# glmanhtu/vit-ed

Hardware: AMD Instinct MI355X
Metric: patch-pairs/sec fwd+bwd, div2k_erosion7_4bin_patch8_64 ViT-ED (higher is better)
Workload: dtype bf16

## Files before the change

### include/vited.h

```cpp
#ifndef VITED_H
#define VITED_H

#include <stdint.h>

#ifdef __cplusplus
extern "C" {
#endif

#define VITED_ABI_VERSION 1

#define VITED_OK 0
#define VITED_ERR_BAD_ARG 1
#define VITED_ERR_UNSUPPORTED 2
#define VITED_ERR_LAUNCH 3
#define VITED_ERR_WORKSPACE 4

#define VITED_F32 0
#define VITED_BF16 1
#define VITED_F16 2
#define VITED_I32 3
#define VITED_I64 4

#define VITED_EPI_STORE 0
#define VITED_EPI_GELU 1
// ... 112 lines not shown
int vited_qk_norm_fwd(const void* q, int64_t q_ld, int64_t q_rows, const void* k, int64_t k_ld, int64_t k_rows,
                      const float* gamma_q, const float* beta_q, const float* gamma_k, const float* beta_k, void* q_out,
                      int64_t q_out_ld, void* k_out, int64_t k_out_ld, float* q_mean, float* q_rstd, float* k_mean,
                      float* k_rstd, int dtype, int64_t heads, int64_t head_dim, float eps, void* stream);

int64_t vited_qk_norm_bwd_workspace_bytes(int64_t q_rows, int64_t k_rows, int64_t heads, int64_t head_dim);
int vited_qk_norm_bwd(void* dq, int64_t dq_ld, const void* q, int64_t q_ld, const float* q_mean, const float* q_rstd,
                      const float* gamma_q, float* dgamma_q, float* dbeta_q, int64_t q_rows, void* dk, int64_t dk_ld,
                      const void* k, int64_t k_ld, const float* k_mean, const float* k_rstd, const float* gamma_k,
                      float* dgamma_k, float* dbeta_k, int64_t k_rows, int dtype, int accumulate, int64_t heads,
                      int64_t head_dim, float* workspace, int64_t workspace_bytes, void* stream);


int64_t vited_token_pool_workspace_bytes(int64_t items, int64_t tokens, int64_t first, int64_t dim);
int vited_token_pool_fwd(const float* x, int64_t x_is, int64_t x_ts, const float* gamma, const float* beta, float eps,
                         float* pooled, int64_t pooled_ld, float* mean, float* rstd, int64_t items, int64_t tokens,
                         int64_t first, int64_t dim, float* workspace, int64_t workspace_bytes, void* stream);

int vited_token_pool_bwd(const float* g, int64_t g_ld, const float* x, int64_t x_is, int64_t x_ts, const float* gamma,
                         const float* mean, const float* rstd, float* dx, int64_t dx_is, int64_t dx_ts, void* dx_lp,
                         int dx_lp_dtype, int64_t dx_lp_is, int64_t dx_lp_ts, const float* lp_scale, float* dgamma,
                         float* dbeta, int accumulate, int64_t items, int64_t tokens, int64_t first, int64_t dim,
                         float* workspace, int64_t workspace_bytes, void* stream);


int vited_gemm(const void* A, int64_t lda, const void* B, int64_t ldb, int b_layout, int dtype, int64_t M,
               int64_t N, int64_t K, int epilogue, const float* bias, const void* aux,
               const float* residual, void* out, void* out2, int64_t ldo, int64_t rows_per_batch,
               int64_t out_rows_per_batch, int64_t row_offset, int residual_bcast, void* stream);

int vited_gemm_scaled(const void* A, int64_t lda, const void* B, int64_t ldb, int b_layout, int dtype, int64_t M, int64_t N,
                      int64_t K, const float* bias, const float* residual, const float* row_scale, float* out, int64_t ldo,
                      void* stream);

int64_t vited_linear_bwd_weight_workspace_bytes(int64_t M, int64_t N, int64_t K);
int vited_linear_bwd_weight(const void* dY, int64_t lddy, const void* X, int64_t ldx, int dtype, int64_t M,
                            int64_t N, int64_t K, float* dW, float* dbias, int accumulate, float* workspace,
                            int64_t workspace_bytes, void* stream);

int vited_linear_bwd_weight_batched_supported(int count, const int64_t* M, const int64_t* N, const int64_t* K, int dtype);
int64_t vited_linear_bwd_weight_batched_workspace_bytes(int count, const int64_t* M, const int64_t* N, const int64_t* K);
int vited_linear_bwd_weight_batched(int count, const void* const* dY, const int64_t* lddy, const void* const* X,
                                    const int64_t* ldx, const int64_t* M, const int64_t* N, const int64_t* K, float* const* dW,
                                    float* const* dbias, int dtype, int accumulate, float* workspace, int64_t workspace_bytes,
                                    void* stream);

int vited_linear_layernorm_supported(int64_t M, int64_t N, int64_t K);

int vited_linear_residual_layernorm_fwd(const void* a, int64_t lda, const void* w, int64_t ldw, const float* bias,
                                        const float* residual, int64_t ldr, float* y, int64_t ldy, const float* gamma,
                                        const float* beta, float eps, void* h, int64_t ldh, float* mean, float* rstd,
                                        int64_t M, int64_t N, int64_t K, void* stream);

int vited_linear_residual_layernorm_fwd_scaled(const void* a, int64_t lda, const void* w, int64_t ldw, const float* bias,
                                               const float* residual, int64_t ldr, const float* row_scale, float* y, int64_t ldy,
                                               const float* gamma, const float* beta, float eps, void* h, int64_t ldh, float* mean,
                                               float* rstd, int64_t M, int64_t N, int64_t K, void* stream);

int vited_linear_layernorm_bwd_segmented(const void* dy, int64_t lddy, int64_t seg_k, int64_t seg_stride, int64_t segments,
                                         const void* wt, int64_t ldwt, const float* x, int64_t ldx, const float* gamma,
                                         const float* mean, const float* rstd, const float* dx_in, int64_t dx_in_ld,
                                         float* dx_out, int64_t dx_out_ld, void* dx_lp, int64_t dx_lp_ld, float* dgamma,
                                         float* dbeta, int accumulate, int64_t M, int64_t N, float* workspace,
                                         int64_t workspace_bytes, void* stream);
int64_t vited_linear_layernorm_bwd_partial_rows(int64_t M);
int64_t vited_linear_layernorm_bwd_partial_rows_n(int64_t M, int64_t N);
// ... 202 lines not shown
```

### vit-ed_amd/csrc/gemm.hip

```cpp
#include <stdlib.h>
#include <string.h>

#include "gemm_kernels.h"

static thread_local int g_last_gemm_path = 0;
extern "C" int vited_last_gemm_path(void) { return g_last_gemm_path; }

static thread_local int g_last_fp32_gemm_kernel = 0;
static int g_fp32_gemm_select = 0;
extern "C" int vited_last_fp32_gemm_kernel(void) { return g_last_fp32_gemm_kernel; }
extern "C" int vited_fp32_gemm_select(int mode) {
    if (mode != 0 && mode != 1) return VITED_ERR_BAD_ARG;
    return __atomic_exchange_n(&g_fp32_gemm_select, mode, __ATOMIC_RELAXED);
}
extern "C" int vited_gemm_f32_mfma_supported(int64_t M, int64_t N, int64_t K, int b_layout, int epilogue) {
    if (M <= 0 || N <= 0 || K <= 0 || epilogue < VITED_EPI_STORE || epilogue > VITED_EPI_GELU_GRAD) return 0;
    return gemm_f32_mfma_supported(M, N, K, b_layout, epilogue) ? 1 : 0;
}
static inline bool fp32_gemm_on_matrix_cores(int64_t M, int64_t N, int64_t K, int b_layout, int epilogue) {
    return __atomic_load_n(&g_fp32_gemm_select, __ATOMIC_RELAXED) == 0 && gemm_f32_mfma_supported(M, N, K, b_layout, epilogue);
}

static int gemm_impl(const void* A, int64_t lda, const void* B, int64_t ldb, int b_layout, int dtype, int64_t M, int64_t N, int64_t K,
                     int epilogue, const float* bias, const void* aux, const float* residual, void* out, void* out2, int64_t ldo,
// ... 21 lines not shown
    ep.out2 = out2;
    ep.ldo = ldo;
    ep.rows_per_batch = epilogue == VITED_EPI_RESIDUAL ? rows_per_batch : 0;
    ep.out_rows_per_batch = out_rows_per_batch;
    ep.row_offset = row_offset;
    ep.residual_bcast = residual_bcast;
    hipStream_t s = (hipStream_t)stream;
    if (dtype == VITED_BF16 && b_layout == VITED_B_NK && gemm_nt_mfma_supported(A, lda, B, ldb, M, N, K, epilogue, ep)) {
        g_last_gemm_path = 2;
        return gemm_nt_mfma(A, lda, B, ldb, M, N, K, epilogue, ep, s);
    }
    g_last_gemm_path = 1;
    if (fp32_gemm_on_matrix_cores(M, N, K, b_layout, epilogue)) {
        g_last_fp32_gemm_kernel = 2;
        return gemm_f32_mfma(A, lda, B, ldb, b_layout, dtype, M, N, K, epilogue, ep, s);
    }
    g_last_fp32_gemm_kernel = 1;
    return gemm_portable(A, lda, B, ldb, b_layout, dtype, M, N, K, epilogue, ep, s);
}

extern "C" int vited_gemm(const void* A, int64_t lda, const void* B, int64_t ldb, int b_layout, int dtype, int64_t M,
                          int64_t N, int64_t K, int epilogue, const float* bias, const void* aux, const float* residual,
                          void* out, void* out2, int64_t ldo, int64_t rows_per_batch, int64_t out_rows_per_batch,
                          int64_t row_offset, int residual_bcast, void* stream) {
    return gemm_impl(A, lda, B, ldb, b_layout, dtype, M, N, K, epilogue, bias, aux, residual, out, out2, ldo, rows_per_batch,
                     out_rows_per_batch, row_offset, residual_bcast, nullptr, stream);
}

extern "C" int vited_gemm_scaled(const void* A, int64_t lda, const void* B, int64_t ldb, int b_layout, int dtype, int64_t M,
                                 int64_t N, int64_t K, const float* bias, const float* residual, const float* row_scale,
                                 float* out, int64_t ldo, void* stream) {
    return gemm_impl(A, lda, B, ldb, b_layout, dtype, M, N, K, VITED_EPI_RESIDUAL, bias, nullptr, residual, out, nullptr, ldo, 0, 0, 0, 0,
                     row_scale, stream);
}

static inline int64_t tn_portable_splits(int64_t M, int64_t N, int64_t K) {
    const int64_t tiles = ceil_div64(N, 64) * ceil_div64(K, 64);
    int64_t s = ceil_div64(1024, tiles);
    const int64_t max_s = ceil_div64(M, 256);
    if (s > max_s) s = max_s;
    if (s < 1) s = 1;
    const int64_t rps = ceil_div64(ceil_div64(M, s), 16) * 16;
    return ceil_div64(M, rps);
}

static inline int64_t max64(int64_t a, int64_t b) { return a > b ? a : b; }

extern "C" int64_t vited_linear_bwd_weight_workspace_bytes(int64_t M, int64_t N, int64_t K) {
    const int64_t s = max64(tn_portable_splits(M, N, K), gemm_tn_mfma_splits(M, N, K));
    return (s * N * K + s * N + N) * (int64_t)sizeof(float) + vited_sum_rows_workspace_bytes(M, N) + 256;
}

extern "C" int vited_linear_bwd_weight(const void* dY, int64_t lddy, const void* X, int64_t ldx, int dtype, int64_t M,
                                       int64_t N, int64_t K, float* dW, float* dbias, int accumulate, float* workspace,
                                       int64_t workspace_bytes, void* stream) {
    if (!dY || !X || !dW || M <= 0 || N <= 0 || K <= 0 || lddy < N || ldx < K) return VITED_ERR_BAD_ARG;
    if (dtype != VITED_F32 && dtype != VITED_BF16) return VITED_ERR_UNSUPPORTED;
    if (!workspace || workspace_bytes < vited_linear_bwd_weight_workspace_bytes(M, N, K)) return VITED_ERR_WORKSPACE;
    hipStream_t s = (hipStream_t)stream;
    const bool mfma = dtype == VITED_BF16 && gemm_tn_mfma_supported(dY, lddy, X, ldx, M, N, K);
    const int64_t splits = mfma ? gemm_tn_mfma_splits(M, N, K) : tn_portable_splits(M, N, K);
    const bool via_slabs = splits > 1 || accumulate;
    float* slab = via_slabs ? workspace : dW;
    float* bias_tmp = workspace + splits * N * K;
    int rc;
    if (mfma) {
// ... 74 lines not shown
```

### vit-ed_amd/csrc/gemm_kernels.h

```cpp
#pragma once
#include "gemm_epilogue.h"

int gemm_portable(const void* A, int64_t lda, const void* B, int64_t ldb, int b_layout, int dtype, int64_t M, int64_t N,
                  int64_t K, int epilogue, const EpiParams& ep, hipStream_t s);
int gemm_tn_portable(const void* dY, int64_t lddy, const void* X, int64_t ldx, int dtype, int64_t M, int64_t N, int64_t K,
                     int64_t splits, float* out, hipStream_t s);

bool gemm_f32_mfma_supported(int64_t M, int64_t N, int64_t K, int b_layout, int epilogue);
int gemm_f32_mfma(const void* A, int64_t lda, const void* B, int64_t ldb, int b_layout, int dtype, int64_t M, int64_t N,
                  int64_t K, int epilogue, const EpiParams& ep, hipStream_t s);
int gemm_tn_f32_mfma(const void* dY, int64_t lddy, const void* X, int64_t ldx, int dtype, int64_t M, int64_t N, int64_t K,
                     int64_t splits, float* out, hipStream_t s);

bool gemm_nt_mfma_supported(const void* A, int64_t lda, const void* B, int64_t ldb, int64_t M, int64_t N, int64_t K,
                            int epilogue, const EpiParams& ep);
int gemm_nt_mfma(const void* A, int64_t lda, const void* B, int64_t ldb, int64_t M, int64_t N, int64_t K, int epilogue,
                 const EpiParams& ep, hipStream_t s);
bool gemm_nt_areg_supported(int64_t ldw, int64_t M, int64_t N, int64_t K, int epilogue);
int gemm_nt_areg(const void* A, int64_t lda, const void* W, int64_t ldw, int64_t M, int64_t N, int epilogue, int waves,
                 const EpiParams& ep, hipStream_t s);
bool gemm_tn_mfma_supported(const void* dY, int64_t lddy, const void* X, int64_t ldx, int64_t M, int64_t N, int64_t K);
int64_t gemm_tn_mfma_splits(int64_t M, int64_t N, int64_t K);
int gemm_tn_mfma(const void* dY, int64_t lddy, const void* X, int64_t ldx, int64_t M, int64_t N, int64_t K, int64_t splits,
                 float* out, float* bias_out , hipStream_t s);

bool gemm_tn_batch_supported(int count, const int64_t* M, const int64_t* N, const int64_t* K);
void gemm_tn_batch_layout(int count, const int64_t* M, const int64_t* N, const int64_t* K, int64_t* splits, int64_t* slab_stride,
                          int64_t* bias_stride);
int gemm_tn_batch(int count, const void* const* dY, const int64_t* lddy, const void* const* X, const int64_t* ldx, const int64_t* M,
                  const int64_t* N, const int64_t* K, const int* has_bias, float* slabs, float* bias_slabs, hipStream_t s);
int sum_slabs_batch(int count, const float* slabs, int64_t slab_stride, const float* bias_slabs, int64_t bias_stride, int64_t splits,
                    const int64_t* widths, float* const* dW, const int64_t* nbias, float* const* dbias, int accumulate, hipStream_t s);

int sum_rows_f32_single_pass(const float* in, int64_t in_ld, float* out, int64_t batch, int64_t width, hipStream_t s,
                             int accumulate = 0);
int sum_slabs_pair(const float* in_a, int64_t ld_a, float* out_a, int64_t width_a, const float* in_b, int64_t ld_b, float* out_b,
                   int64_t width_b, int64_t batch, hipStream_t s, int accumulate);
```

### vit-ed_amd/csrc/gemm_mfma.hip

```cpp
#include <stdlib.h>

#include <mutex>

#include "gemm_kernels.h"
#include "gemm_nt_epilogue.h"
#include "gemm_lds.h"

template <int BKT, int WM, bool ASM_DMA = false>
__device__ __forceinline__ void nt_stage_load(const bf16* __restrict__ A, int64_t lda, const bf16* __restrict__ B,
                                              int64_t ldb, int64_t m0, int64_t n0, int64_t M, int64_t N, int64_t k0,
                                              char* stage, int wave, int lane) {
    using C = NtCfg<BKT, WM>;
    const int rsub = lane / C::CHUNKS, cp = lane % C::CHUNKS;
#ifndef NT_DBG_NO_A_DMA
#pragma unroll
    for (int i = 0; i < 32 / C::ROWS_PER_DMA; ++i) {
        const int r = wave * 32 + i * C::ROWS_PER_DMA + rsub;
        const int c = cp ^ C::swz(r);
        int64_t gm = m0 + r;
        gm = gm < M ? gm : M - 1;
        const bf16* asrc = A + gm * lda + k0 + c * 8;
        if constexpr (ASM_DMA) glds16_asm(asrc, stage + (wave * 32 + i * C::ROWS_PER_DMA) * C::ROW_BYTES);
        else glds16(asrc, stage + (wave * 32 + i * C::ROWS_PER_DMA) * C::ROW_BYTES);
    }
// ... 154 lines not shown
    if (ceil_div64(M, 128) * ceil_div64(N, BN) > (1 << 30)) return false;
    if (M >= ((int64_t)1 << 31) || ep.rows_per_batch >= ((int64_t)1 << 31)) return false;
    return true;
}

template <int EPI, int BKT, int WM, int STAGES = 2>
static int launch_nt(const bf16* a, int64_t lda, const bf16* b, int64_t ldb, int64_t M, int64_t N, int64_t K, const EpiParams& ep,
                      hipStream_t s) {
    using C = NtCfg<BKT, WM>;
    const int tiles_n = (int)ceil_div64(N, BN);
    const int ntiles = (int)ceil_div64(M, C::BM) * tiles_n;
    auto kernel = gemm_nt_mfma_kernel<EPI, BKT, WM, STAGES>;
    constexpr int LDS = STAGES * C::STAGE_BYTES;
    if (LDS > 65536) {
        static std::once_flag once;
        static hipError_t status = hipSuccess;
        std::call_once(once, [&] { status = hipFuncSetAttribute((const void*)kernel, hipFuncAttributeMaxDynamicSharedMemorySize, LDS); });
        if (status != hipSuccess) return VITED_ERR_LAUNCH;
    }
    hipLaunchKernelGGL(kernel, dim3(ntiles), dim3(128 * WM), LDS, s, a, lda, b, ldb, M, N, K, tiles_n, ntiles, ep);
    return VITED_OK;
}

template <int EPI> static inline int nt_areg_waves(int64_t ldb, int64_t M, int64_t N, int64_t K) {
    if (!gemm_nt_areg_supported(ldb, M, N, K, EPI)) return 0;
#ifdef VITED_TUNING
    if (const char* force = getenv("VITED_NT_AREG")) return atoi(force);
#endif
    if (EPI == VITED_EPI_MUL) return 8;
    if (EPI == VITED_EPI_STORE && N >= 1152 && M >= 65536) return 4;
    return 0;
}

template <int EPI>
static int dispatch_nt(const bf16* a, int64_t lda, const bf16* b, int64_t ldb, int64_t M, int64_t N, int64_t K, const EpiParams& ep,
                       hipStream_t s) {
    if (const int waves = nt_areg_waves<EPI>(ldb, M, N, K)) return gemm_nt_areg(a, lda, b, ldb, M, N, EPI, waves, ep, s);
    bool shallow = K <= 512 && N >= 768;
    constexpr bool tall_epi = EPI == VITED_EPI_STORE || EPI == VITED_EPI_MUL || EPI == VITED_EPI_GELU_GRAD;
    bool tall = tall_epi && shallow && N >= 768 && M >= 8192;
#ifdef VITED_TUNING
    static const int force_bk = getenv("VITED_NT_BK") ? atoi(getenv("VITED_NT_BK")) : 0;
    static const int force_wm = getenv("VITED_NT_WM") ? atoi(getenv("VITED_NT_WM")) : 0;
    static const int force_st = getenv("VITED_NT_STAGES") ? atoi(getenv("VITED_NT_STAGES")) : 0;
    if (force_bk) shallow = force_bk == 32;
    if (force_wm) tall = force_wm == 4;
    if (force_st == 3) {
        if (shallow && tall) return launch_nt<EPI, 32, 4, 3>(a, lda, b, ldb, M, N, K, ep, s);
        if (shallow) return launch_nt<EPI, 32, 2, 3>(a, lda, b, ldb, M, N, K, ep, s);
        if (tall) return launch_nt<EPI, 64, 4, 3>(a, lda, b, ldb, M, N, K, ep, s);
        return launch_nt<EPI, 64, 2, 3>(a, lda, b, ldb, M, N, K, ep, s);
    }
#endif
    if (shallow && tall && EPI == VITED_EPI_STORE) return launch_nt<EPI, 32, 4, 3>(a, lda, b, ldb, M, N, K, ep, s);
    if (shallow && tall) return launch_nt<EPI, 32, 4>(a, lda, b, ldb, M, N, K, ep, s);
    if (shallow) return launch_nt<EPI, 32, 2>(a, lda, b, ldb, M, N, K, ep, s);
    if (tall) return launch_nt<EPI, 64, 4>(a, lda, b, ldb, M, N, K, ep, s);
    return launch_nt<EPI, 64, 2>(a, lda, b, ldb, M, N, K, ep, s);
}

int gemm_nt_mfma(const void* A, int64_t lda, const void* B, int64_t ldb, int64_t M, int64_t N, int64_t K, int epilogue,
                 const EpiParams& ep, hipStream_t s) {
    const bf16* a = (const bf16*)A;
    const bf16* b = (const bf16*)B;
    int rc;
    switch (epilogue) {
        case VITED_EPI_STORE: rc = dispatch_nt<VITED_EPI_STORE>(a, lda, b, ldb, M, N, K, ep, s); break;
        case VITED_EPI_GELU: rc = dispatch_nt<VITED_EPI_GELU>(a, lda, b, ldb, M, N, K, ep, s); break;
        case VITED_EPI_RESIDUAL: rc = dispatch_nt<VITED_EPI_RESIDUAL>(a, lda, b, ldb, M, N, K, ep, s); break;
// ... 623 lines not shown
```

### vit-ed_amd/functions.py

```python
from __future__ import annotations

import contextlib
import os
from collections import namedtuple

import torch

from . import ops
from ._lib import (B_KN, B_NK, EPI_GELU_GRAD, EPI_MUL, EPI_RESIDUAL, EPI_STORE, EPI_STORE_F32)
from .shadows import WeightShadows

LN_EPS = 1e-6


def _bundle(name, table):
    fields, keys = zip(*(pair.split('=') for pair in table.split()))
    return namedtuple(name, fields), keys


_ATTN = 'g1=norm1.weight b1=norm1.bias wqkv=attn.qkv.weight bqkv=attn.qkv.bias wproj=attn.proj.weight bproj=attn.proj.bias '
_CROSS = ('gc=norm_cross.weight bc=norm_cross.bias gx=norm_context.weight bx=norm_context.bias wq=cross_attn.q.weight '
          'bq=cross_attn.q.bias wkv=cross_attn.kv.weight bkv=cross_attn.kv.bias wcp=cross_attn.proj.weight bcp=cross_attn.proj.bias ')
_MLP = 'g2=norm2.weight b2=norm2.bias w1=mlp.fc1.weight bb1=mlp.fc1.bias w2=mlp.fc2.weight bb2=mlp.fc2.bias'
_PATCH = 'pw=patch_embed.proj.weight pb=patch_embed.proj.bias pos=pos_embed '
# ... 40 lines not shown
    _step_hook_installed = True


class Runtime:

    def __init__(self, *, img_size, patch_size, in_chans, num_classes, embed_dim, depth, c_depth, num_heads,
                 act_dtype=torch.bfloat16, qk_norm=False, global_pool='token', fc_norm=False):
        if global_pool not in ('token', 'avg'):
            raise NotImplementedError(f'global_pool={global_pool!r}: the head pools the cls token (\'token\') or averages the patch tokens (\'avg\')')
        self.pool_avg, self.fc_norm = global_pool == 'avg', bool(fc_norm)
        self.dec_shared = DecSharedFc if self.fc_norm else DecShared
        self.qk_norm = bool(qk_norm)
        self.enc_block, self.dec_block = (EncBlockQK, DecBlockQK) if self.qk_norm else (EncBlock, DecBlock)
        self.img_size, self.patch_size, self.in_chans = img_size, patch_size, in_chans
        self.num_classes, self.dim, self.depth, self.c_depth, self.heads = num_classes, embed_dim, depth, c_depth, num_heads
        self.n1 = (img_size // patch_size) ** 2
        self.n2 = self.n1 + 1
        self.head_dim = embed_dim // num_heads
        self.scale = self.head_dim ** -0.5
        self.act_dtype = act_dtype
        self.direct_grads = False
        self.input_mean, self.input_std = (0.5, 0.5, 0.5), (0.5, 0.5, 0.5)
        self.keep_attn = False
        self.keep_cam = False
        self.attn_store = {}
        self.cls_tail = os.environ.get('VITED_CLS_TAIL', '1') != '0' and not self.pool_avg
        self.fused_mlp = os.environ.get('VITED_FUSED_MLP', '1') != '0'
        self.fused_ln = os.environ.get('VITED_FUSED_LN', '1') != '0'
        self.batch_dw = os.environ.get('VITED_BATCH_DW', '1') != '0'
        self.group_dw = os.environ.get('VITED_GROUP_DW', '1') != '0'
        self.dw_queue = None
        self.ln_queue = None
        self.fold_context = os.environ.get('VITED_FOLD_CONTEXT', '1') != '0'
        self._fold_bufs = None
        self._unit_ln = None
        self.tap = None
        self.block_events = None
        self.shadows = WeightShadows()
        if not self.exact:
            _install_optimizer_step_hook()

    @property
    def exact(self):
        return self.act_dtype == torch.float32

    def weight(self, w: torch.Tensor) -> torch.Tensor:
        w2 = w.detach().reshape(w.shape[0], -1)
        if self.exact:
            return w2
        return self.shadows.get(w, 'n', lambda out=None: ops.cast(w2, self.act_dtype, out=out))

    def weight_t(self, w: torch.Tensor):
        w2 = w.detach().reshape(w.shape[0], -1)
        if self.exact:
            return w2, B_KN
        return self.shadows.get(w, 't', lambda out=None: ops.cast_transpose(w2.contiguous(), self.act_dtype, out=out)), B_NK

    def refresh_shadows(self, params):
        self.shadows.refresh(params)


def shadows_of(model):
    return [rt.shadows for rt in getattr(model, '_runtimes', {}).values()]


class _BlockSpan:
# ... 684 lines not shown
        if l == 0 and q0 is not None:
            xa, q = x, q0.index_select(0, j_idx)
        else:
            xa, _, lnq = _dec_self_fwd(rt, x, P, batch, n, cls_only, fuse_ln=not cls_only)
        xb, _, _ = _dec_cross_fwd(rt, xa, P, batch, lnq=lnq, q=q, kv3=kv3, kv_index=i_idx, fuse_ln=False)
        x, _, _ = _mlp_fwd(rt, xb, P, grad=False)
    return _head_fwd(rt, x, shared, batch, n, rt.cls_tail and rt.c_depth > 0, save=False)[0]


def _kv_params(blocks):
    return [P.wkv for P in blocks], [P.bkv for P in blocks], [P.gx for P in blocks], [P.bx for P in blocks]


FoldSaved = namedtuple('FoldSaved', 'kv_all xhat mean rstd wt')
FinalSaved = namedtuple('FinalSaved', 'xcls y mean rstd')
PoolSaved = namedtuple('PoolSaved', 'x y mean rstd')


def _context_kv_folded(rt, ctxf, blocks):
    dev = ctxf.device
    if rt._unit_ln is None or rt._unit_ln[0].device != dev:
        rt._unit_ln = (torch.ones(rt.dim, dtype=torch.float32, device=dev), torch.zeros(rt.dim, dtype=torch.float32, device=dev))
    ws, bs, gs, bes = _kv_params(blocks)
    bufs = rt._fold_bufs
    if bufs is not None and (bufs[0].shape[0] != len(blocks) * 2 * rt.dim or bufs[0].device != dev):
        rt.shadows.retire(bufs)
        bufs = None
    rt._fold_bufs = bufs = ops.fold_context_weights([w.detach() for w in ws], [b.detach() if b is not None else None for b in bs],
                                                    [g.detach() for g in gs], [b.detach() for b in bes], out=bufs)
    xhat, mean, rstd = ops.layernorm_fwd(ctxf, rt._unit_ln[0], rt._unit_ln[1], LN_EPS, rt.act_dtype)
    n2 = 2 * rt.dim
    kv_all = torch.empty((len(blocks), ctxf.shape[0], n2), dtype=rt.act_dtype, device=dev)
    wf, wft, bf = bufs
    for l in range(len(blocks)):
        ops.gemm(xhat, wf[l * n2:(l + 1) * n2], bias=bf[l * n2:(l + 1) * n2], out=kv_all[l])
    return FoldSaved(kv_all, xhat, mean, rstd, wt=wft)


def _context_kv_folded_bwd(rt, dkv_all, ctxf, saved, blocks):
    xhat, wt = saved.xhat, saved.wt
    ones = rt._unit_ln[0]
    nblk, mc, n2 = dkv_all.shape
    if _row_kernel_ok(rt, mc, wt.shape[0], nblk * n2, dkv_all.dtype, ctxf):
        dctx, _, _, _ = ops.linear_layernorm_bwd(dkv_all, wt, ctxf, ones, saved.mean, saved.rstd)
    else:
        dh = torch.zeros((mc, rt.dim), dtype=torch.float32, device=ctxf.device)
        for l in range(nblk):
            dh = ops.gemm(dkv_all[l], wt[:, l * n2:(l + 1) * n2], epilogue=EPI_RESIDUAL, residual=dh)
        dctx, _, _, _ = ops.layernorm_bwd(dh, ctxf, ones, saved.mean, saved.rstd)
    dwf = torch.empty((nblk * n2, rt.dim), dtype=torch.float32, device=ctxf.device)
    dbf = torch.empty(nblk * n2, dtype=torch.float32, device=ctxf.device)
    _launch_weight_grads([(dkv_all[l], xhat, dwf[l * n2:(l + 1) * n2], dbf[l * n2:(l + 1) * n2]) for l in range(nblk)], False)
    ws, bs, gs, bes = _kv_params(blocks)
    targets = [(_gtarget(rt, w), _gtarget(rt, b) if b is not None else None, _gtarget(rt, g), _gtarget(rt, be)) for w, b, g, be in zip(ws, bs, gs, bes)]
    direct = all(tw is not None and tg is not None and tbe is not None and (b is None or tb is not None) for (tw, tb, tg, tbe), b in zip(targets, bs))
    if not direct:
        targets = [(torch.empty_like(w), torch.empty_like(b) if b is not None else None, torch.empty_like(g), torch.empty_like(be))
                   for w, b, g, be in zip(ws, bs, gs, bes)]
    ops.unfold_context_grads(dwf, dbf, [w.detach() for w in ws], [g.detach() for g in gs], [b.detach() for b in bes],
                             [tw for tw, _, _, _ in targets], [tb for _, tb, _, _ in targets], [tg for _, _, tg, _ in targets],
                             [tbe for _, _, _, tbe in targets], accumulate=direct)
    return dctx, [dict.fromkeys(('gx', 'bx', 'wkv', 'bkv')) if direct else dict(gx=tg, bx=tbe, wkv=tw, bkv=tb) for tw, tb, tg, tbe in targets]


def _head_fwd(rt, x, S, batch, n, cls_rows, save=True):
    d = rt.dim
# ... 151 lines not shown
```

### vit-ed_amd/ops.py

```python
from __future__ import annotations

import contextlib
import ctypes as C
from typing import NamedTuple

import torch

from . import _lib
from ._lib import (B_KN, B_NK, BF16, EPI_GELU, EPI_GELU_GRAD, EPI_MUL, EPI_MUL_GELU_GRAD, EPI_RESIDUAL, EPI_STORE, EPI_STORE_F32, F16,
                   F32, I32, I64)

_DTYPE = {torch.float32: F32, torch.bfloat16: BF16, torch.float16: F16, torch.int32: I32, torch.int64: I64}
_FLOATS = (torch.float32, torch.bfloat16, torch.float16)
_ACT = (torch.float32, torch.bfloat16)


def _code(dtype: torch.dtype) -> int:
    if dtype not in (torch.float32, torch.bfloat16):
        raise TypeError(f'vited ops support float32 and bfloat16 activations, got {dtype}')
    return _DTYPE[dtype]


def _need_gpu(*tensors, error=RuntimeError):
    for t in tensors:
# ... 1096 lines not shown
              _stream())


from .ops_patchdrop import (MAX_KEEP_KEYS, keep_from_keys, keep_inverse, patchify_kept, tokens_kept,
                            tokens_kept_bwd)

from .ops_poolhead import POOL_MAX_DIM, token_pool_bwd, token_pool_fwd

from .ops_tokendrop import (TOKEN_DROPOUT_MAX_DIM, dropout_threshold, philox4x32, token_dropout,
                            token_dropout_mask)

from .ops_lrsched import LR_MAX_MILESTONES, LR_TABLE_WORDS, lr_schedule_step

from .ops_lrfinder import (LRF_DIVERGED, LRF_DONE, LRF_HISTORY_COLS, LRF_NONFINITE, LRF_RUNNING, LRF_STATE_WORDS,
                           lr_finder_rate, lr_finder_step, lr_suggestion)

from .ops_minedloss import MINED_BCE_MAX_CLASSES, mined_bce

from .ops_ranklists import TOPK_MAX_K, retrieval_curve_rows, retrieval_topk_rows

from .ops_puzzlepixels import (PUZZLE_MAX_ERODED, PUZZLE_MAX_PIECES, PUZZLE_MAX_SIZE, puzzle_assemble, puzzle_cut,
                               puzzle_eroded_width, puzzle_pixel_distances, puzzle_resize_pieces)

from .ops_puzzle2 import (puzzle_assemble2, puzzle_best_slot2, puzzle_compat2_init, puzzle_compat2_recalc,
                          puzzle_pixel_distances2, puzzle_unpack_slot2)

from .ops_puzzlerot import patchify_turned, puzzle_distances2_from_logits

from .ops_puzzlemixed import puzzle_mutual_gather

from .ops_ema import ema_swap

from .ops_f32attn import fp32_attention_kernels, fp32_attention_supported, last_fp32_attention_kernel
```

Baseline: 44350.

## Add weight-in-register persistent NT GEMM for K=384 bf16 projections

```diff
diff --git a/include/vited.h b/include/vited.h
--- a/include/vited.h
+++ b/include/vited.h
@@ -168,6 +168,11 @@
 int vited_gemm_scaled(const void* A, int64_t lda, const void* B, int64_t ldb, int b_layout, int dtype, int64_t M, int64_t N,
                       int64_t K, const float* bias, const float* residual, const float* row_scale, float* out, int64_t ldo,
                       void* stream);
+
+int vited_gemm_nt_wreg_supported(int64_t lda, int64_t ldw, int64_t ldo, int64_t M, int groups, int groups_inner, int64_t group_stride);
+int vited_gemm_nt_wreg(const void* A, int64_t lda, const void* W, int64_t ldw, const float* bias, void* out, int64_t ldo, int64_t M,
+                       int groups, int groups_inner, int64_t group_stride, int workgroups, void* stream);
+int vited_gemm_nt_wreg_select(int mode);
 
 int64_t vited_linear_bwd_weight_workspace_bytes(int64_t M, int64_t N, int64_t K);
 int vited_linear_bwd_weight(const void* dY, int64_t lddy, const void* X, int64_t ldx, int dtype, int64_t M,
diff --git a/profiles/wreg_probe.py b/profiles/wreg_probe.py
--- /dev/null
+++ b/profiles/wreg_probe.py
@@ -0,0 +1,98 @@
+#!/usr/bin/env python3
+import argparse
+import json
+import os
+import statistics
+import sys
+
+import torch
+
+sys.path.insert(0, os.path.dirname(os.path.dirname(os.path.abspath(__file__))))
+import vited_amd as v
+
+ops = v.ops
+K = W = 384
+COLD_BYTES = 1 << 30
+
+
+def main():
+    ap = argparse.ArgumentParser()
+    ap.add_argument('--rows', type=int, nargs='+', default=[24576, 65536, 66560, 73800])
+    ap.add_argument('--rounds', type=int, default=7)
+    ap.add_argument('--reps', type=int, default=40)
+    ap.add_argument('--json', default=None)
+    a = ap.parse_args()
+    dev = torch.device('cuda:0')
+    g = torch.Generator(device=dev).manual_seed(0)
+
+    def rnd(*shape, scale=1.0):
+        return torch.randn(*shape, generator=g, device=dev) * scale
+
+    def arms_for(M, sets):
+        xs = [rnd(M, K).bfloat16() for _ in range(sets)]
+        w16, b16 = rnd(16 * W, K, scale=0.05).bfloat16(), rnd(16 * W)
+        o1 = [torch.empty(M, W, device=dev, dtype=torch.bfloat16) for _ in range(sets)]
+        kv = [torch.empty(8, M, 2 * W, device=dev, dtype=torch.bfloat16) for _ in range(sets)]
+        o3 = [torch.empty(M, 3 * W, device=dev, dtype=torch.bfloat16) for _ in range(sets)]
+
+        def tile(i, bias):
+            with ops.gemm_nt_wreg_dispatch(False):
+                ops.gemm(xs[i], w16[:W], bias=b16[:W] if bias else None, out=o1[i])
+
+        def kv_loop(i):
+            with ops.gemm_nt_wreg_dispatch(False):
+                for l in range(8):
+                    ops.gemm(xs[i], w16[l * 2 * W:(l + 1) * 2 * W], bias=b16[l * 2 * W:(l + 1) * 2 * W], out=kv[i][l])
+
+        def qkv_old(i):
+            with ops.gemm_nt_wreg_dispatch(False):
+                ops.gemm(xs[i], w16[:3 * W], bias=b16[:3 * W], out=o3[i])
+
+        return {
+            'n384+bias': (lambda i: tile(i, True), lambda i: ops.gemm_nt_wreg(xs[i], w16[:W], b16[:W], o1[i])),
+            'n384': (lambda i: tile(i, False), lambda i: ops.gemm_nt_wreg(xs[i], w16[:W], None, o1[i])),
+            'kv 8x768': (kv_loop, lambda i: ops.gemm_nt_wreg(xs[i], w16, b16, kv[i])),
+            'qkv 1152': (qkv_old, lambda i: ops.gemm_nt_wreg(xs[i], w16[:3 * W], b16[:3 * W], o3[i])),
+        }
+
+    results = []
+    for M in a.rows:
+        for label, sets in (('warm', 1), ('cold', max(2, -(-COLD_BYTES // (M * (K + W) * 2))))):
+            arms = arms_for(M, sets)
+            print(f'M = {M} {label} ({sets} buffer set{"s" if sets > 1 else ""}; us: median [min .. max] over {a.rounds} rounds of {a.reps})')
+            for name, pair in arms.items():
+                times, graphs = ([], []), []
+                for fn in pair:
+                    for i in range(min(sets, 3)):
+                        fn(i)
+                    torch.cuda.synchronize()
+                    graph = torch.cuda.CUDAGraph()
+                    with torch.cuda.graph(graph):
+                        for r in range(a.reps):
+                            fn(r % sets)
+                    graph.replay()
+                    graphs.append(graph)
+                torch.cuda.synchronize()
+                for _ in range(a.rounds):
+                    for which, graph in enumerate(graphs):
+                        e0, e1 = torch.cuda.Event(enable_timing=True), torch.cuda.Event(enable_timing=True)
+                        e0.record()
+                        graph.replay()
+                        e1.record()
+                        torch.cuda.synchronize()
+                        times[which].append(e0.elapsed_time(e1) / a.reps * 1e3)
+                line = f'  {name:10s}'
+                for which, t in zip(('old', 'new'), times):
+                    line += f' | {which}: {statistics.median(t):7.1f} [{min(t):7.1f} .. {max(t):7.1f}]'
+                    results.append(dict(M=M, cache=label, shape=name, arm=which, us=[round(x, 2) for x in t]))
+                print(line, flush=True)
+                del graphs
+            del arms
+            torch.cuda.empty_cache()
+    if a.json:
+        with open(a.json, 'w') as f:
+            json.dump(results, f, indent=0)
+
+
+if __name__ == '__main__':
+    main()
diff --git a/vit-ed_amd/csrc/gemm.hip b/vit-ed_amd/csrc/gemm.hip
--- a/vit-ed_amd/csrc/gemm.hip
+++ b/vit-ed_amd/csrc/gemm.hip
@@ -77,6 +77,24 @@
                                  float* out, int64_t ldo, void* stream) {
     return gemm_impl(A, lda, B, ldb, b_layout, dtype, M, N, K, VITED_EPI_RESIDUAL, bias, nullptr, residual, out, nullptr, ldo, 0, 0, 0, 0,
                      row_scale, stream);
+}
+
+static int g_nt_wreg_select = 0;
+bool gemm_nt_wreg_auto() { return __atomic_load_n(&g_nt_wreg_select, __ATOMIC_RELAXED) == 0; }
+extern "C" int vited_gemm_nt_wreg_select(int mode) {
+    if (mode != 0 && mode != 1) return VITED_ERR_BAD_ARG;
+    return __atomic_exchange_n(&g_nt_wreg_select, mode, __ATOMIC_RELAXED);
+}
+extern "C" int vited_gemm_nt_wreg_supported(int64_t lda, int64_t ldw, int64_t ldo, int64_t M, int groups, int groups_inner,
+                                            int64_t group_stride) {
+    return gemm_nt_wreg_supported(lda, ldw, ldo, M, groups, groups_inner, group_stride) ? 1 : 0;
+}
+extern "C" int vited_gemm_nt_wreg(const void* A, int64_t lda, const void* W, int64_t ldw, const float* bias, void* out, int64_t ldo,
+                                  int64_t M, int groups, int groups_inner, int64_t group_stride, int workgroups, void* stream) {
+    if (!A || !W || !out || workgroups < 0) return VITED_ERR_BAD_ARG;
+    const int rc = gemm_nt_wreg(A, lda, W, ldw, bias, out, ldo, M, groups, groups_inner, group_stride, workgroups, (hipStream_t)stream);
+    if (rc == VITED_OK) g_last_gemm_path = 2;
+    return rc;
 }
 
 static inline int64_t tn_portable_splits(int64_t M, int64_t N, int64_t K) {
diff --git a/vit-ed_amd/csrc/gemm_kernels.h b/vit-ed_amd/csrc/gemm_kernels.h
--- a/vit-ed_amd/csrc/gemm_kernels.h
+++ b/vit-ed_amd/csrc/gemm_kernels.h
@@ -19,6 +19,10 @@
 bool gemm_nt_areg_supported(int64_t ldw, int64_t M, int64_t N, int64_t K, int epilogue);
 int gemm_nt_areg(const void* A, int64_t lda, const void* W, int64_t ldw, int64_t M, int64_t N, int epilogue, int waves,
                  const EpiParams& ep, hipStream_t s);
+bool gemm_nt_wreg_supported(int64_t lda, int64_t ldw, int64_t ldo, int64_t M, int groups, int groups_inner, int64_t group_stride);
+int gemm_nt_wreg(const void* A, int64_t lda, const void* W, int64_t ldw, const float* bias, void* out, int64_t ldo, int64_t M,
+                 int groups, int groups_inner, int64_t group_stride, int workgroups, hipStream_t s);
+bool gemm_nt_wreg_auto();
 bool gemm_tn_mfma_supported(const void* dY, int64_t lddy, const void* X, int64_t ldx, int64_t M, int64_t N, int64_t K);
 int64_t gemm_tn_mfma_splits(int64_t M, int64_t N, int64_t K);
 int gemm_tn_mfma(const void* dY, int64_t lddy, const void* X, int64_t ldx, int64_t M, int64_t N, int64_t K, int64_t splits,
diff --git a/vit-ed_amd/csrc/gemm_mfma.hip b/vit-ed_amd/csrc/gemm_mfma.hip
--- a/vit-ed_amd/csrc/gemm_mfma.hip
+++ b/vit-ed_amd/csrc/gemm_mfma.hip
@@ -210,9 +210,27 @@
     return 0;
 }
 
+#ifndef NT_WREG_MIN_M
+#define NT_WREG_MIN_M 32768
+#endif
+#ifndef NT_WREG_QKV_MIN_M
+#define NT_WREG_QKV_MIN_M 65536
+#endif
+static inline int nt_wreg_groups(int64_t lda, int64_t ldb, int64_t M, int64_t N, int64_t K, const EpiParams& ep) {
+    if (K != 384 || !gemm_nt_wreg_auto()) return 0;
+    int groups = 0;
+    if (N == 384 && M >= (int64_t)NT_WREG_MIN_M) groups = 1;
+    if (N == 1152 && NT_WREG_QKV_MIN_M > 0 && M >= (int64_t)NT_WREG_QKV_MIN_M) groups = 3;
+    return groups && gemm_nt_wreg_supported(lda, ldb, ep.ldo, M, groups, groups, 0) ? groups : 0;
+}
+
 template <int EPI>
 static int dispatch_nt(const bf16* a, int64_t lda, const bf16* b, int64_t ldb, int64_t M, int64_t N, int64_t K, const EpiParams& ep,
                        hipStream_t s) {
+    if constexpr (EPI == VITED_EPI_STORE) {
+        if (const int groups = nt_wreg_groups(lda, ldb, M, N, K, ep))
+            return gemm_nt_wreg(a, lda, b, ldb, ep.bias, ep.out, ep.ldo, M, groups, groups, 0, 0, s);
+    }
     if (const int waves = nt_areg_waves<EPI>(ldb, M, N, K)) return gemm_nt_areg(a, lda, b, ldb, M, N, EPI, waves, ep, s);
     bool shallow = K <= 512 && N >= 768;
     constexpr bool tall_epi = EPI == VITED_EPI_STORE || EPI == VITED_EPI_MUL || EPI == VITED_EPI_GELU_GRAD;
diff --git a/vit-ed_amd/csrc/gemm_nt_wreg.hip b/vit-ed_amd/csrc/gemm_nt_wreg.hip
--- /dev/null
+++ b/vit-ed_amd/csrc/gemm_nt_wreg.hip
@@ -0,0 +1,165 @@
+#include <mutex>
+
+#include "gemm_kernels.h"
+#include "gemm_lds.h"
+#include "gemm_nt_wreg_split.h"
+
+#define WREG_KSTEPS 12
+#define WREG_N 384
+#define WREG_TILE_ROWS (2 * WREG_UNIT_ROWS)
+#define WREG_CHUNK_BYTES (WREG_TILE_ROWS * 128)
+#define WREG_TILE_BYTES (6 * WREG_CHUNK_BYTES)
+#define WREG_SLOTS 5
+#define WREG_STAGE_LD 784
+#define WREG_STAGE_BYTES (WREG_TILE_ROWS * WREG_STAGE_LD)
+#define WREG_LDS_BYTES (WREG_SLOTS * WREG_TILE_BYTES + WREG_STAGE_BYTES)
+#define WREG_SLOTS_RESIDENT 256
+
+__global__ void __launch_bounds__(512) __attribute__((amdgpu_waves_per_eu(2, 2)))
+gemm_nt_wreg_kernel(const bf16* __restrict__ A, int64_t lda, const bf16* __restrict__ W, int64_t ldw, const float* __restrict__ bias,
+                    bf16* __restrict__ out, int64_t ldo, int64_t M, int per, int units, int groups_inner, int64_t group_stride) {
+    extern __shared__ __attribute__((aligned(16))) char smem[];
+    using C = NtCfg<64>;
+    constexpr int S = WREG_SLOTS;
+    const int lane = threadIdx.x & 63;
+    const int wave = __builtin_amdgcn_readfirstlane(threadIdx.x >> 6);
+    const int fr = lane & 15, fq = lane >> 4;
+
+    const WregShare sh = wreg_share((int)blockIdx.x, per, units);
+    if (sh.unit_begin >= sh.unit_end) return;
+    const int64_t row_begin = (int64_t)sh.unit_begin * WREG_UNIT_ROWS;
+    const int64_t row_stop = (int64_t)sh.unit_end * WREG_UNIT_ROWS;
+    const int64_t row_end = row_stop < M ? row_stop : M;
+    const int nsteps = (sh.unit_end - sh.unit_begin + 1) >> 1;
+
+    int arow[3], acol[3];
+#pragma unroll
+    for (int j = 0; j < 3; ++j) {
+        const int p = wave * 3 + j;
+        arow[j] = (p & 3) * 8 + (lane >> 3);
+        acol[j] = (p >> 2) * 64 + (((lane & 7) ^ C::swz(arow[j])) << 3);
+    }
+    auto issue = [&](int t, int slot) {
+        const int64_t r0 = row_begin + (int64_t)t * WREG_TILE_ROWS;
+        char* dst = smem + slot * WREG_TILE_BYTES + wave * 3 * 1024;
+#pragma unroll
+        for (int j = 0; j < 3; ++j) {
+            int64_t gm = r0 + arow[j];
+            gm = gm < M ? gm : M - 1;
+            glds16_asm(A + gm * lda + acol[j], dst + j * 1024);
+        }
+    };
+#pragma unroll
+    for (int p = 0; p < S - 1; ++p)
+        if (p < nsteps) issue(p, p);
+
+    bf16x8 w[3][WREG_KSTEPS];
+    float bv[3];
+#pragma unroll
+    for (int j = 0; j < 3; ++j) {
+        const int n = sh.group * WREG_N + wave * 48 + j * 16 + fr;
+        const bf16* wrow = W + (int64_t)n * ldw + fq * 8;
+#pragma unroll
+        for (int ks = 0; ks < WREG_KSTEPS; ++ks) w[j][ks] = *(const bf16x8*)(wrow + ks * 32);
+        bv[j] = bias ? bias[n] : 0.f;
+    }
+    __builtin_amdgcn_s_waitcnt(0x0f70);
+
+    int aoff[2];
+#pragma unroll
+    for (int kk = 0; kk < 2; ++kk) aoff[kk] = C::off(fr, kk * 4 + fq);
+    char* stage = smem + S * WREG_TILE_BYTES;
+    char* swr = stage + (fq * 4) * WREG_STAGE_LD + (wave * 48 + fr) * 2;
+    int srow[3], scol[3];
+#pragma unroll
+    for (int jj = 0; jj < 3; ++jj) {
+        const int q = (int)threadIdx.x + 512 * jj;
+        srow[jj] = q / 48;
+        scol[jj] = q - srow[jj] * 48;
+    }
+    bf16* outg = out + (int64_t)(sh.group / groups_inner) * group_stride + (int64_t)(sh.group % groups_inner) * WREG_N;
+
+    int slot = 0, islot = S - 1;
+    for (int t = 0; t < nsteps; ++t) {
+        const int left = nsteps - 1 - t;
+        if (left >= S - 2) asm volatile("s_waitcnt vmcnt(%0) lgkmcnt(0)" ::"n"(3 * (S - 2)) : "memory");
+        else if (left == 2) asm volatile("s_waitcnt vmcnt(6) lgkmcnt(0)" ::: "memory");
+        else if (left == 1) asm volatile("s_waitcnt vmcnt(3) lgkmcnt(0)" ::: "memory");
+        else asm volatile("s_waitcnt vmcnt(0) lgkmcnt(0)" ::: "memory");
+        __builtin_amdgcn_s_barrier();
+        asm volatile("" ::: "memory");
+        if (t + S - 1 < nsteps) issue(t + S - 1, islot);
+
+        const char* sa = smem + slot * WREG_TILE_BYTES;
+        f32x4 acc[2][3];
+#pragma unroll
+        for (int i = 0; i < 2; ++i)
+#pragma unroll
+            for (int j = 0; j < 3; ++j) acc[i][j] = f32x4{0.f, 0.f, 0.f, 0.f};
+        bf16x8 af[2][2][2];
+        auto read4 = [&](int buf, int kc) {
+#pragma unroll
+            for (int kk = 0; kk < 2; ++kk)
+#pragma unroll
+                for (int i = 0; i < 2; ++i)
+                    af[buf][kk][i] = *(const bf16x8*)(sa + kc * WREG_CHUNK_BYTES + i * (16 * C::ROW_BYTES) + aoff[kk]);
+        };
+        read4(0, 0);
+#pragma unroll
+        for (int kc = 0; kc < 6; ++kc) {
+            if (kc + 1 < 6) read4((kc + 1) & 1, kc + 1);
+            __builtin_amdgcn_sched_barrier(0);
+#pragma unroll
+            for (int kk = 0; kk < 2; ++kk)
+#pragma unroll
+                for (int j = 0; j < 3; ++j)
+#pragma unroll
+                    for (int i = 0; i < 2; ++i)
+                        acc[i][j] = __builtin_amdgcn_mfma_f32_16x16x32_bf16(af[kc & 1][kk][i], w[j][kc * 2 + kk], acc[i][j], 0, 0, 0);
+            __builtin_amdgcn_sched_barrier(0);
+        }
+
+#pragma unroll
+        for (int i = 0; i < 2; ++i)
+#pragma unroll
+            for (int j = 0; j < 3; ++j)
+#pragma unroll
+                for (int e = 0; e < 4; ++e)
+                    *(bf16*)(swr + (i * 16 + e) * WREG_STAGE_LD + j * 32) = (bf16)(acc[i][j][e] + bv[j]);
+        asm volatile("s_waitcnt lgkmcnt(0)" ::: "memory");
+        __builtin_amdgcn_s_barrier();
+        asm volatile("" ::: "memory");
+        const int64_t r0 = row_begin + (int64_t)t * WREG_TILE_ROWS;
+#pragma unroll
+        for (int jj = 0; jj < 3; ++jj) {
+            const bf16x8 v = *(const bf16x8*)(stage + srow[jj] * WREG_STAGE_LD + scol[jj] * 16);
+            const int64_t m = r0 + srow[jj];
+            if (m < row_end) *(bf16x8*)(outg + m * ldo + scol[jj] * 8) = v;
+        }
+        slot = slot + 1 == S ? 0 : slot + 1;
+        islot = islot + 1 == S ? 0 : islot + 1;
+    }
+}
+
+bool gemm_nt_wreg_supported(int64_t lda, int64_t ldw, int64_t ldo, int64_t M, int groups, int groups_inner, int64_t group_stride) {
+    if (M < 1 || M >= ((int64_t)1 << 31) || groups < 1 || groups > 4096 || groups_inner < 1 || group_stride < 0) return false;
+    if (lda < 32 * WREG_KSTEPS || ldw < 32 * WREG_KSTEPS || ldo < (int64_t)WREG_N * groups_inner) return false;
+    return lda % 8 == 0 && ldw % 8 == 0 && ldo % 8 == 0 && group_stride % 8 == 0;
+}
+
+int gemm_nt_wreg(const void* A, int64_t lda, const void* W, int64_t ldw, const float* bias, void* out, int64_t ldo, int64_t M,
+                 int groups, int groups_inner, int64_t group_stride, int workgroups, hipStream_t s) {
+    if (workgroups < 0) return VITED_ERR_BAD_ARG;
+    if (!gemm_nt_wreg_supported(lda, ldw, ldo, M, groups, groups_inner, group_stride)) return VITED_ERR_UNSUPPORTED;
+    if (((uintptr_t)A | (uintptr_t)W | (uintptr_t)out) & 15 || (uintptr_t)bias & 3) return VITED_ERR_BAD_ARG;
+    static std::once_flag once;
+    static hipError_t status = hipSuccess;
+    std::call_once(once, [&] {
+        status = hipFuncSetAttribute((const void*)gemm_nt_wreg_kernel, hipFuncAttributeMaxDynamicSharedMemorySize, WREG_LDS_BYTES);
+    });
+    if (status != hipSuccess) return VITED_ERR_LAUNCH;
+    const int per = wreg_per_group(workgroups ? workgroups : WREG_SLOTS_RESIDENT, groups);
+    hipLaunchKernelGGL(gemm_nt_wreg_kernel, dim3(per * groups), dim3(512), WREG_LDS_BYTES, s, (const bf16*)A, lda, (const bf16*)W, ldw,
+                       bias, (bf16*)out, ldo, M, per, (int)wreg_units(M), groups_inner, group_stride);
+    return vited_check_launch();
+}
diff --git a/vit-ed_amd/csrc/gemm_nt_wreg_split.h b/vit-ed_amd/csrc/gemm_nt_wreg_split.h
--- /dev/null
+++ b/vit-ed_amd/csrc/gemm_nt_wreg_split.h
@@ -0,0 +1,32 @@
+#pragma once
+#include <stdint.h>
+
+#if defined(__HIPCC__)
+#define WREG_FN __host__ __device__ __forceinline__
+#else
+#define WREG_FN inline
+#endif
+
+#define WREG_UNIT_ROWS 16
+
+struct WregShare {
+    int group;
+    int unit_begin;
+    int unit_end;
+};
+
+WREG_FN int64_t wreg_units(int64_t M) { return (M + WREG_UNIT_ROWS - 1) / WREG_UNIT_ROWS; }
+
+WREG_FN int wreg_per_group(int workgroups, int groups) {
+    const int per = workgroups / groups;
+    return per < 1 ? 1 : per;
+}
+
+WREG_FN WregShare wreg_share(int wg, int per, int64_t units) {
+    WregShare s;
+    s.group = wg / per;
+    const int64_t i = wg - s.group * per;
+    s.unit_begin = (int)(i * units / per);
+    s.unit_end = (int)((i + 1) * units / per);
+    return s;
+}
diff --git a/vit-ed_amd/functions.py b/vit-ed_amd/functions.py
--- a/vit-ed_amd/functions.py
+++ b/vit-ed_amd/functions.py
@@ -96,6 +96,7 @@
         self.dw_queue = None
         self.ln_queue = None
         self.fold_context = os.environ.get('VITED_FOLD_CONTEXT', '1') != '0'
+        self.kv_one_launch = os.environ.get('VITED_KV_ONE_LAUNCH', '0') != '0'
         self._fold_bufs = None
         self._unit_ln = None
         self.tap = None
@@ -846,6 +847,10 @@
     n2 = 2 * rt.dim
     kv_all = torch.empty((len(blocks), ctxf.shape[0], n2), dtype=rt.act_dtype, device=dev)
     wf, wft, bf = bufs
+    if (rt.kv_one_launch and rt.dim == ops.WREG_WIDTH and xhat.dtype == torch.bfloat16
+            and ops.gemm_nt_wreg_supported(xhat.shape[0], 2 * len(blocks), 2, lda=xhat.stride(0), ldw=wf.stride(0))):
+        ops.gemm_nt_wreg(xhat, wf, bf, kv_all, groups=2 * len(blocks))
+        return FoldSaved(kv_all, xhat, mean, rstd, wt=wft)
     for l in range(len(blocks)):
         ops.gemm(xhat, wf[l * n2:(l + 1) * n2], bias=bf[l * n2:(l + 1) * n2], out=kv_all[l])
     return FoldSaved(kv_all, xhat, mean, rstd, wt=wft)
diff --git a/vit-ed_amd/ops.py b/vit-ed_amd/ops.py
--- a/vit-ed_amd/ops.py
+++ b/vit-ed_amd/ops.py
@@ -1152,3 +1152,5 @@
 from .ops_ema import ema_swap
 
 from .ops_f32attn import fp32_attention_kernels, fp32_attention_supported, last_fp32_attention_kernel
+
+from .ops_wreg import WREG_WIDTH, gemm_nt_wreg, gemm_nt_wreg_dispatch, gemm_nt_wreg_supported
diff --git a/vit-ed_amd/ops_wreg.py b/vit-ed_amd/ops_wreg.py
--- /dev/null
+++ b/vit-ed_amd/ops_wreg.py
@@ -0,0 +1,58 @@
+from __future__ import annotations
+
+import contextlib
+
+import torch
+
+from . import ops as _o
+
+_f32, _bf16 = torch.float32, torch.bfloat16
+WREG_WIDTH = 384
+
+
+def gemm_nt_wreg_supported(m: int, groups: int, groups_inner: int = 1, lda: int = WREG_WIDTH, ldw: int = WREG_WIDTH,
+                           ldo: int | None = None, group_stride: int | None = None) -> bool:
+    ldo = WREG_WIDTH * groups_inner if ldo is None else ldo
+    group_stride = m * ldo if group_stride is None else group_stride
+    return bool(_o._lib.load().vited_gemm_nt_wreg_supported(int(lda), int(ldw), int(ldo), int(m), int(groups), int(groups_inner),
+                                                             int(group_stride)))
+
+
+def gemm_nt_wreg(a: torch.Tensor, w: torch.Tensor, bias=None, out=None, *, groups: int | None = None, workgroups: int = 0):
+    _o._need_gpu(a, w, bias, out)
+    op, dev = 'gemm_nt_wreg', a.device
+    lda = _o._rows(op, 'a', a, _bf16, dev, cols=WREG_WIDTH)
+    m = a.shape[0]
+    ldw = _o._rows(op, 'w', w, _bf16, dev, cols=WREG_WIDTH, like='a')
+    g = w.shape[0] // WREG_WIDTH
+    if g < 1 or w.shape[0] != g * WREG_WIDTH or (groups is not None and groups != g):
+        raise ValueError(f'{op}: w has {w.shape[0]} rows, which are not {"whole" if groups is None else groups} groups of {WREG_WIDTH}')
+    if out is None:
+        out = torch.empty((m, g * WREG_WIDTH), dtype=_bf16, device=dev)
+    if torch.is_tensor(out) and out.dim() == 3:
+        _o._check(op, 'out', out, _bf16, (None, m, None), dev, _o.DENSE_LAST)
+        outer, width, ldo, group_stride = out.shape[0], out.shape[2], out.stride(1), out.stride(0) if out.shape[0] > 1 else 0
+    else:
+        _o._check(op, 'out', out, _bf16, (m, None), dev, _o.DENSE_LAST)
+        outer, width, ldo, group_stride = 1, out.shape[1], out.stride(0), 0
+    inner = width // WREG_WIDTH
+    if inner < 1 or width != inner * WREG_WIDTH or outer * inner != g:
+        raise ValueError(f'{op}: out {list(out.shape)} does not hold {g} groups of {WREG_WIDTH} columns')
+    if m == 1:
+        lda, ldo = max(lda, WREG_WIDTH), max(ldo, width)
+    _o._check(op, 'bias', bias, _f32, g * WREG_WIDTH, dev, optional=True)
+    if workgroups < 0:
+        raise ValueError(f'{op}: workgroups must be >= 0, got {workgroups}')
+    _o._lib.call('vited_gemm_nt_wreg', _o._ptr(a), lda, _o._ptr(w), ldw, _o._ptr(bias), _o._ptr(out), ldo, m, g, inner, group_stride,
+                 int(workgroups), _o._stream())
+    return out
+
+
+@contextlib.contextmanager
+def gemm_nt_wreg_dispatch(enabled: bool):
+    select = _o._lib.load().vited_gemm_nt_wreg_select
+    previous = select(0 if enabled else 1)
+    try:
+        yield
+    finally:
+        select(previous)
```

After: 45010, median of 6. +1.5%, better.
